# m96-chan/PyGPUkit

Measured on AMD Instinct MI355X. Metric: decode tokens/sec/GPU + prefill TFLOPS (% MFMA peak), Qwen3-0.6B bf16, higher is better.
Workload: dtype bf16

## Files before the change

include/pgk_hip.h:

```cpp
#ifndef PGK_HIP_H
#define PGK_HIP_H

#include <stddef.h>
#include <stdint.h>

#ifdef __cplusplus
extern "C" {
#endif

typedef int pgk_status;
#define PGK_OK 0
#define PGK_ERR_INVALID 1
#define PGK_ERR_HIP 2
#define PGK_ERR_UNSUPPORTED 3
#define PGK_ERR_RCCL 4
#define PGK_ERR_JIT 5

typedef enum {
    PGK_F64 = 0, PGK_F32 = 1, PGK_F16 = 2, PGK_BF16 = 3, PGK_I64 = 4,
    PGK_I32 = 5, PGK_I16 = 6, PGK_I8 = 7, PGK_U8 = 8, PGK_I4 = 9
} pgk_dtype;

typedef void* pgk_stream;
typedef void* pgk_event;
// ... 154 lines not shown
                             pgk_stream s);
pgk_status pgk_gemm_fp8_nt(const uint8_t* a_fp8, const float* a_scale, const uint8_t* w_fp8_nk, const void* w_scale,
                           void* c, int m, int n, int k, pgk_stream s);
pgk_status pgk_gemm_fp8_fp8_nn(const uint8_t* a_mk, const uint8_t* b_kn, uint8_t* d_mn, const float* scale_a,
                               const float* scale_b, int m, int n, int k, pgk_stream s);
pgk_status pgk_quantize_fp8_rows(const void* x, uint8_t* out_fp8, float* out_scale, int m, int k, pgk_dtype dt,
                                 pgk_stream s);
pgk_status pgk_quantize_fp8_blocks(const void* w_bf16, uint8_t* out_fp8, void* out_scale_bf16, int n, int k,
                                   pgk_stream s);

pgk_status pgk_quantize_nvf4(const void* x_kn, uint8_t* data, uint8_t* scale, int k, int n, pgk_stream s);
pgk_status pgk_quantize_nvf4_nk(const void* x_nk, uint8_t* data, uint8_t* scale, int n, int k, pgk_stream s);
size_t pgk_gemv_nvf4_workspace_bytes(int k, int n);
pgk_status pgk_gemv_nvf4_bf16(const void* a, const uint8_t* data, const uint8_t* scale, void* c, void* workspace, int k,
                              int n, float alpha, pgk_stream s);
pgk_status pgk_quantize_e2m1_unit(const void* x, uint8_t* out, int rows, int k, int transpose, pgk_stream s);
pgk_status pgk_gemm_fp4_nt(const uint8_t* a_packed, const uint8_t* b_packed, void* d, int m, int n, int kp, pgk_stream s);
size_t pgk_gemm_nvf4_workspace_bytes(int m, int n, int k);

pgk_status pgk_sdpa_causal(const void* q, const void* k, const void* v, void* out, int hq, int hkv, int q_len,
                           int kv_len, int d, float scale, int64_t q_stride_h, int64_t q_stride_s,
                           int64_t kv_stride_h, int64_t kv_stride_s, int64_t o_stride_h, int64_t o_stride_s,
                           pgk_dtype dt, pgk_stream s);
pgk_status pgk_sdpa_causal_fp8(const void* q, const void* k, const void* v, void* out, int hq, int hkv, int q_len,
                               int kv_len, int d, float scale, int64_t q_stride_h, int64_t q_stride_s,
                               int64_t kv_stride_h, int64_t kv_stride_s, int64_t o_stride_h, int64_t o_stride_s,
                               pgk_dtype dt, pgk_stream s);
pgk_status pgk_quantize_fp8_per_head(const void* x, uint8_t* codes, uint8_t* scale_bytes, int heads, int rows, int d,
                                     int64_t stride_h, int64_t stride_s, pgk_dtype dt, pgk_stream s);
pgk_status pgk_l2norm(const void* in, void* out, int rows, int features, float eps, pgk_dtype dt, pgk_stream s);
pgk_status pgk_irope_scale_q(const void* q, const void* positions, void* out, int seq_len, int n_heads, int head_dim,
                             float attn_scale, float floor_scale, pgk_dtype pos_dt, pgk_dtype dt, pgk_stream s);
pgk_status pgk_sdpa_irope(const void* q, const void* k, const void* v, const void* positions, void* out, int hq, int hkv,
                          int q_len, int kv_len, int d, float attn_scale, float floor_scale, int causal_offset,
                          int64_t q_stride_h, int64_t q_stride_s, int64_t kv_stride_h, int64_t kv_stride_s,
                          int64_t o_stride_h, int64_t o_stride_s, pgk_dtype pos_dt, pgk_dtype dt, pgk_stream s);
pgk_status pgk_llama4_qk_norm_cache_write(void* q, const void* k, const void* v, void* k_cache, void* v_cache, int seq, int hq,
                                          int hkv, int max_seq, int d, float eps, int qk_norm, int h_pos,
                                          const int32_t* pos_buf, pgk_dtype dt, pgk_stream s);
pgk_status pgk_sdpa_irope_fixed_cache(const void* q, const void* k_cache, const void* v_cache, void* out, int hq, int hkv,
                                      int max_seq, int d, float attn_scale, float floor_scale, int h_pos,
                                      const int32_t* pos_buf, void* workspace, pgk_dtype dt, pgk_stream s);
pgk_status pgk_pope_inplace(void* q, void* k, const void* encoding, int seq, int hq, int hk, int d, int start_pos, int max_seq,
                            pgk_dtype dt, pgk_stream s);
pgk_status pgk_alibi_compute_bias(const void* slopes, void* bias, int seq_len, int num_heads, int causal, pgk_stream s);
pgk_status pgk_alibi_add_bias(void* scores, const void* slopes, int batch, int num_heads, int q_len, int kv_len, int start_pos,
// ... 88 lines not shown
```

pygpukit_amd/_hip.py:

```python

from __future__ import annotations

import ctypes as C
import os

_HERE = os.path.dirname(os.path.abspath(__file__))
LIB_PATH = os.environ.get("PGK_LIB") or os.path.join(_HERE, "libpgk_hip.so")

c_void_pp = C.POINTER(C.c_void_p)
c_i32_p = C.POINTER(C.c_int32)


class PgkError(RuntimeError):
    """A libpgk_hip call returned a non-zero status (reference: std::runtime_error / CudaError
    surfacing as RuntimeError, native/core/types.hpp:108-111)."""


class DeviceProps(C.Structure):
    _fields_ = [("name", C.c_char * 128), ("arch", C.c_char * 32), ("total_mem", C.c_size_t),
                ("cu_count", C.c_int), ("wavefront_size", C.c_int), ("clock_khz", C.c_int),
                ("lds_per_cu", C.c_int), ("l2_bytes", C.c_int)]


class PoolStats(C.Structure):
# ... 47 lines not shown
    "pgk_argmax": [_V, _I, _I, _I, _V, _V],
    "pgk_gemm_nn": [_V, _V, _V, _I, _I, _I, _I, _V], "pgk_gemm_nt": [_V, _V, _V, _V, _I, _I, _I, _I, _V],
    "pgk_gemv": [_V, _V, _V, _I, _I, _I, _V], "pgk_gemv_fp8_bf16": [_V, _V, _V, _V, _I, _I, _I, _V],
    "pgk_w8a16_gemm_kn": [_V, _V, _V, _V, _I, _I, _I, _V], "pgk_w8a16_gemm_nk": [_V, _V, _V, _V, _I, _I, _I, _V],
    "pgk_gemm_fp8_nt": [_V, _V, _V, _V, _V, _I, _I, _I, _V], "pgk_gemm_fp8_fp8_nn": [_V, _V, _V, _V, _V, _I, _I, _I, _V],
    "pgk_quantize_fp8_rows": [_V, _V, _V, _I, _I, _I, _V],
    "pgk_quantize_fp8_blocks": [_V, _V, _V, _I, _I, _V],
    "pgk_quantize_nvf4": [_V, _V, _V, _I, _I, _V], "pgk_quantize_nvf4_nk": [_V, _V, _V, _I, _I, _V], "pgk_gemv_nvf4_bf16": [_V, _V, _V, _V, _V, _I, _I, _F, _V],
    "pgk_quantize_e2m1_unit": [_V, _V, _I, _I, _I, _V], "pgk_gemm_fp4_nt": [_V, _V, _V, _I, _I, _I, _V],
    "pgk_paged_attention_v1": [_V, _V, _V, _V, _V, _V, _I, _I, _I, _I, _I, _I, _I, _F, _V, _I, _V],
    "pgk_paged_cache_write": [_V, _V, _V, _V, _V, _I, _I, _I, _I, _I, _V],
    "pgk_scatter_last_token_logits": [_V, _V, _V, _V, _I, _I, _I, _V], "pgk_prepare_position_ids": [_V, _V, _V, _V, _V, _I, _V],
    "pgk_check_eos": [_V, _V, _I, _I, _V], "pgk_exclusive_cumsum_i32": [_V, _V, _I, _V],
    "pgk_st_open": [C.c_char_p, c_void_pp],
    "pgk_st_tensor_info": [_V, C.c_char_p, C.POINTER(_I), C.POINTER(_I), C.POINTER(_I64), C.POINTER(C.c_uint64), C.POINTER(C.c_uint64)],
    "pgk_st_tensor_data": [_V, C.c_char_p, c_void_pp, C.POINTER(C.c_uint64)], "pgk_st_upload": [_V, C.c_char_p, _V, C.c_uint64, _V],
    "pgk_jit_version": [C.POINTER(_I), C.POINTER(_I)],
    "pgk_jit_compile": [C.c_char_p, C.c_char_p, C.POINTER(C.c_char_p), _I, c_void_pp, C.POINTER(_I)],
    "pgk_jit_program_code": [_V, c_void_pp, C.POINTER(_Z)], "pgk_jit_kernel_create": [_V, C.c_char_p, c_void_pp, C.POINTER(_I)],
    "pgk_jit_suggested_block_size": [_V, _Z, C.POINTER(_I)],
    "pgk_jit_launch": [_V, C.c_uint, C.c_uint, C.c_uint, C.c_uint, C.c_uint, C.c_uint, C.c_uint, c_void_pp, _V],
    "pgk_sample_token": [_V, _I, _I, _I, _F, _I, _F, _F, _V, _V, _V],
    "pgk_sdpa_causal": [_V, _V, _V, _V, _I, _I, _I, _I, _I, _F, _I64, _I64, _I64, _I64, _I64, _I64, _I, _V],
    "pgk_sdpa_causal_fp8": [_V, _V, _V, _V, _I, _I, _I, _I, _I, _F, _I64, _I64, _I64, _I64, _I64, _I64, _I, _V],
    "pgk_quantize_fp8_per_head": [_V, _V, _V, _I, _I, _I, _I64, _I64, _I, _V], "pgk_device_arch": [C.POINTER(_I)],
    "pgk_l2norm": [_V, _V, _I, _I, _F, _I, _V], "pgk_irope_scale_q": [_V, _V, _V, _I, _I, _I, _F, _F, _I, _I, _V],
    "pgk_sdpa_irope": [_V, _V, _V, _V, _V, _I, _I, _I, _I, _I, _F, _F, _I, _I64, _I64, _I64, _I64, _I64, _I64, _I, _I, _V],
    "pgk_llama4_qk_norm_cache_write": [_V, _V, _V, _V, _V, _I, _I, _I, _I, _I, _F, _I, _I, _V, _I, _V],
    "pgk_sdpa_irope_fixed_cache": [_V, _V, _V, _V, _I, _I, _I, _I, _F, _F, _I, _V, _V, _I, _V],
    "pgk_sdpa_fixed_cache": [_V, _V, _V, _V, _I, _I, _I, _I, _I, _F, _I, _V, _V, _I, _V],
    "pgk_pope_inplace": [_V, _V, _V, _I, _I, _I, _I, _I, _I, _I, _V], "pgk_alibi_compute_bias": [_V, _V, _I, _I, _I, _V],
    "pgk_alibi_add_bias": [_V, _V, _I, _I, _I, _I, _I, _I, _I, _I, _V],
    "pgk_sdpa_alibi": [_V, _V, _V, _V, _V, _I, _I, _I, _I, _I, _F, _I64, _I64, _I64, _I64, _I64, _I64, _I, _V],
    "pgk_sdpa_alibi_fixed_cache": [_V, _V, _V, _V, _V, _I, _I, _I, _I, _I, _F, _I, _V, _V, _I, _V],
    "pgk_engine_create": [C.POINTER(ModelConfig), _V, _V, _V, C.POINTER(LayerWeights), c_void_pp],
    "pgk_engine_destroy": [_V], "pgk_engine_bytes": [_V, C.POINTER(_Z), C.POINTER(_Z)],
    "pgk_engine_prefill": [_V, _I, c_i32_p, _I, _I, _V, C.POINTER(_F), _V],
    "pgk_engine_set_state": [_V, c_i32_p, c_i32_p, _I, _V], "pgk_engine_decode_step": [_V, _I, _V],
    "pgk_engine_profile_step": [_V, _I, _I, C.POINTER(_F), C.POINTER(_I), _V],
    "pgk_engine_timeline": [_V, _I, _I, C.POINTER(C.c_uint64), _I, C.POINTER(_I), _V],
    "pgk_engine_capture": [_V, _I, _V], "pgk_engine_replay": [_V, _I, _V], "pgk_engine_logits_ptr": [_V, c_void_pp],
    "pgk_engine_read_tokens": [_V, c_i32_p, _I, _I, _V], "pgk_engine_reset_log": [_V, _V],
    "pgk_engine_set_sampling": [_V, _F, _I, _F, C.POINTER(_F), _I, _V],
    "pgk_engine_read_clock": [_V, C.POINTER(C.c_uint64), _I, _V],
    "pgk_engine_kv_ptr": [_V, _I, c_void_pp, c_void_pp], "pgk_engine_state_ptr": [_V, c_void_pp, c_void_pp], "pgk_engine_launches_per_step": [_V, C.POINTER(_I)],
    "pgk_moe_topk_softmax": [_V, _V, _V, _I, _I, _I, _I, _I, _V], "pgk_moe_softmax_topk": [_V, _I, _I, _I, _V],
# ... 75 lines not shown
```

pygpukit_amd/csrc/flash_common.hip.h:

```cpp
#pragma once

#include <type_traits>

#include "pgk_device.hip.h"
#include "pgk_internal.h"

namespace pgk {

typedef __bf16 bf16x8_fl __attribute__((ext_vector_type(8)));
typedef _Float16 f16x8_fl __attribute__((ext_vector_type(8)));
typedef float f32x16_fl __attribute__((ext_vector_type(16)));

template <class T> __device__ __forceinline__ f32x16_fl mfma32(const uint4& a, const uint4& b, f32x16_fl c);
template <> __device__ __forceinline__ f32x16_fl mfma32<bf16>(const uint4& a, const uint4& b, f32x16_fl c) {
    return __builtin_amdgcn_mfma_f32_32x32x16_bf16(__builtin_bit_cast(bf16x8_fl, a), __builtin_bit_cast(bf16x8_fl, b), c, 0, 0, 0);
}
template <> __device__ __forceinline__ f32x16_fl mfma32<f16>(const uint4& a, const uint4& b, f32x16_fl c) {
    return __builtin_amdgcn_mfma_f32_32x32x16_f16(__builtin_bit_cast(f16x8_fl, a), __builtin_bit_cast(f16x8_fl, b), c, 0, 0, 0);
}
template <class T> __device__ __forceinline__ uint32_t pack16x2(float lo, float hi);
template <> __device__ __forceinline__ uint32_t pack16x2<bf16>(float lo, float hi) { return pack_bf16x2(lo, hi); }
template <> __device__ __forceinline__ uint32_t pack16x2<f16>(float lo, float hi) {
    return (uint32_t)__builtin_bit_cast(uint16_t, static_cast<_Float16>(lo)) | ((uint32_t)__builtin_bit_cast(uint16_t, static_cast<_Float16>(hi)) << 16);
}
// ... 14 lines not shown
}

struct FlashPlain {};
struct FlashIrope {
    const void* positions;
    float attn_scale, floor_scale;
    int causal_offset;
    int pos_is_i64;
};
struct FlashAlibi {
    const float* slopes;
};

__device__ __forceinline__ int fl_v_off(int d, int c8) { return d * 128 + ((c8 ^ ((d >> 1) & 15)) << 3); }

struct FlashSplit {
    int nsplit;
    float* ml;
    void* o;
    uint8_t* q8;
    float* q8s;
};

inline int flash_nsplit(int nqt, int hq, int kv_len) {
    int nsplit = 1, dev = 0, cus = 256;
    hipDeviceProp_t prop;
    if (hipGetDevice(&dev) == hipSuccess && hipGetDeviceProperties(&prop, dev) == hipSuccess && prop.multiProcessorCount > 0) cus = prop.multiProcessorCount;
    const long long wgs = (long long)nqt * hq;
    while (nsplit < 4 && wgs * nsplit < 2LL * cus && ceil_div(kv_len, FL_BKV) >= 4 * (nsplit * 2)) nsplit *= 2;
    return nsplit;
}

template <class T, int D>
__global__ __launch_bounds__(256) void flash_merge_kernel(const float* ml, const T* po, T* out, int hq, int q_len, int nsplit, long long oh, long long os,
                                                          uint8_t* q8 = nullptr, float* q8s = nullptr) {
    constexpr int CPR = D / 8;
    const size_t gid = (size_t)blockIdx.x * 256 + threadIdx.x;
    const size_t nrow = (size_t)q_len * hq;
    if (gid >= nrow * CPR) return;
    const size_t rowi = gid / CPR;
    const int c = (int)(gid % CPR), qrow = (int)(rowi / hq), head = (int)(rowi % hq);
    float mstar = -INFINITY;
    for (int s2 = 0; s2 < nsplit; ++s2) mstar = fmaxf(mstar, ml[(((size_t)s2 * hq + head) * q_len + qrow) * 2]);
    float acc[8] = {0.f, 0.f, 0.f, 0.f, 0.f, 0.f, 0.f, 0.f}, den = 0.f;
    for (int s2 = 0; s2 < nsplit; ++s2) {
        const float* r = ml + (((size_t)s2 * hq + head) * q_len + qrow) * 2;
        const float w = (r[1] > 0.f) ? r[1] * __builtin_amdgcn_exp2f(r[0] - mstar) : 0.f;
        if (w > 0.f) {
            Vec<T> v;
            v.load(po + (((size_t)s2 * q_len + qrow) * hq + head) * D + c * 8);
            float f[8];
            v.to_float(f);
#pragma unroll
// ... 58 lines not shown
```

pygpukit_amd/csrc/ops_flash.hip:

```cpp

#include "flash_common.hip.h"

namespace pgk {

template <int D> __device__ __forceinline__ int fl_k_off(int r, int c) { return r * (2 * D) + ((c ^ (r & (D / 8 - 1))) << 4); }

template <class T, int D, class X = FlashPlain>
__global__ __launch_bounds__(FL_THREADS, 2) void flash_fwd_kernel(const T* q, const T* k, const T* vt, T* out, int hq, int hkv,
                                                              int q_len, int kv_len, int kv_pad, float scale_log2e, FlashStrides sd,
                                                              FlashSplit sp, X ex) {
    constexpr bool IROPE = std::is_same<X, FlashIrope>::value;
    constexpr bool ALIBI = std::is_same<X, FlashAlibi>::value;
    constexpr int NC = D / 8;
    constexpr int KS = D / 16;
    constexpr int DT = D / 32;
    constexpr int KCH = 64 * NC / FL_THREADS;
    constexpr int VCH = D * 8 / FL_THREADS;
    constexpr int K_BYTES = 64 * D * 2, V_BYTES = D * 128;
    extern __shared__ __attribute__((aligned(16))) char fl_smem[];
    auto Ks = [&](int buf) -> char* { return fl_smem + buf * K_BYTES; };
    auto Vs = [&](int buf) -> char* { return fl_smem + 2 * K_BYTES + buf * V_BYTES; };

    const int tid = threadIdx.x, lane = tid & 63, wid = tid >> 6, ql = lane & 31, h = lane >> 5;
    const int rep = hq / hkv, nqt = (q_len + FL_BQ - 1) / FL_BQ;
    const int id = blockIdx.x;
    const int kvh = id % hkv, rest = id / hkv;
    const int head = kvh * rep + rest % rep;
    const int rest2 = rest / rep;
    int order = rest2;
    const int nord = nqt * sp.nsplit;
    if (sp.nsplit > 1 && order >= nord / 2) order = nord / 2 + (nord - 1 - order);
    const int split = order % sp.nsplit;
    const int qt = nqt - 1 - order / sp.nsplit;
    const int qw0 = qt * FL_BQ + wid * 32;
    int mask_off = kv_len - q_len;
    if constexpr (IROPE) mask_off = ex.causal_offset;
    const int causal_off = mask_off;
    const T* qh = q + (size_t)head * sd.qh;
    const T* kh = k + (size_t)kvh * sd.kh;
    const T* vh = vt + (size_t)kvh * D * kv_pad;

    uint4 qf[KS];
    {
        const T* qrow = qh + (size_t)min(qw0 + ql, q_len - 1) * sd.qs + 8 * h;
        float qmul = scale_log2e;
        if constexpr (IROPE)
            qmul *= irope_temperature(irope_position(ex.positions, min(qw0 + ql, q_len - 1), ex.pos_is_i64), ex.attn_scale, ex.floor_scale);
#pragma unroll
        for (int ks = 0; ks < KS; ++ks) {
            Vec<T> v;
            v.load(qrow + ks * 16);
            float f[8];
            v.to_float(f);
#pragma unroll
            for (int j = 0; j < 8; ++j) f[j] *= qmul;
            v.from_float(f);
            qf[ks] = v.raw;
        }
    }
    f32x16_fl o[DT];
#pragma unroll
    for (int i = 0; i < DT; ++i)
#pragma unroll
        for (int r = 0; r < 16; ++r) o[i][r] = 0.f;
    float m_run = -INFINITY, l_run = 0.f;
    float slope2 = 0.f;
    if constexpr (ALIBI) slope2 = ex.slopes[head] * 1.4426950408889634f;

    const int q_last = min(qt * FL_BQ + FL_BQ - 1, q_len - 1);
    const int kv_end = min(kv_len, causal_off + q_last + 1);
    const int nt_all = (kv_end + FL_BKV - 1) / FL_BKV;
    const int t0 = (int)((long long)nt_all * split / sp.nsplit), t1 = (int)((long long)nt_all * (split + 1) / sp.nsplit);

    static_assert(KCH == VCH && (KCH == 2 || KCH == 4), "staging is written for D = 64 / 128");
    uint4 rk0, rk1, rk2, rk3, rv0, rv1, rv2, rv3;
    const int kr = tid / NC, kc16 = tid % NC;
    constexpr int KR_STEP = FL_THREADS / NC;
    const int vd = tid >> 3, vc = tid & 7;
    auto k_src = [&](int kv0, int i) { return kh + (size_t)min(kv0 + kr + KR_STEP * i, kv_len - 1) * sd.ks + kc16 * 8; };
    const uint32_t ko0 = (uint32_t)(kr * sd.ks + kc16 * 8), ko_step = (uint32_t)(KR_STEP * sd.ks);
    const uint32_t vo0 = (uint32_t)(vd * kv_pad + vc * 8), vo_step = (uint32_t)(32 * kv_pad);
    auto load_k = [&](int t) {
        const int kv0 = t * FL_BKV;
        if (kv0 + FL_BKV <= kv_len) {
            const T* kt = kh + (size_t)kv0 * sd.ks;
            rk0 = *reinterpret_cast<const uint4*>(kt + ko0);
            rk1 = *reinterpret_cast<const uint4*>(kt + ko0 + ko_step);
            if constexpr (KCH == 4) {
                rk2 = *reinterpret_cast<const uint4*>(kt + ko0 + 2 * ko_step);
                rk3 = *reinterpret_cast<const uint4*>(kt + ko0 + 3 * ko_step);
            }
        } else {
            rk0 = *reinterpret_cast<const uint4*>(k_src(kv0, 0));
            rk1 = *reinterpret_cast<const uint4*>(k_src(kv0, 1));
            if constexpr (KCH == 4) {
                rk2 = *reinterpret_cast<const uint4*>(k_src(kv0, 2));
                rk3 = *reinterpret_cast<const uint4*>(k_src(kv0, 3));
            }
        }
    };
    auto load_v = [&](int t) {
        const T* vtile = vh + t * FL_BKV;
        rv0 = *reinterpret_cast<const uint4*>(vtile + vo0);
        rv1 = *reinterpret_cast<const uint4*>(vtile + vo0 + vo_step);
        if constexpr (VCH == 4) {
            rv2 = *reinterpret_cast<const uint4*>(vtile + vo0 + 2 * vo_step);
            rv3 = *reinterpret_cast<const uint4*>(vtile + vo0 + 3 * vo_step);
        }
    };
    auto put_v = [&](char* base, int d, const uint4& x) {
        *reinterpret_cast<uint2*>(base + fl_v_off(d, 2 * vc)) = make_uint2(x.x, x.y);
        *reinterpret_cast<uint2*>(base + fl_v_off(d, 2 * vc + 1)) = make_uint2(x.z, x.w);
    };
    auto store_k = [&](int buf) {
        char* kb = Ks(buf);
        *reinterpret_cast<uint4*>(kb + fl_k_off<D>(kr, kc16)) = rk0;
        *reinterpret_cast<uint4*>(kb + fl_k_off<D>(kr + KR_STEP, kc16)) = rk1;
        if constexpr (KCH == 4) {
            *reinterpret_cast<uint4*>(kb + fl_k_off<D>(kr + 2 * KR_STEP, kc16)) = rk2;
            *reinterpret_cast<uint4*>(kb + fl_k_off<D>(kr + 3 * KR_STEP, kc16)) = rk3;
        }
    };
    auto store_v = [&](int buf) {
        char* vb = Vs(buf);
        put_v(vb, vd, rv0);
        put_v(vb, vd + 32, rv1);
        if constexpr (VCH == 4) {
            put_v(vb, vd + 64, rv2);
            put_v(vb, vd + 96, rv3);
        }
    };
    auto qk = [&](int buf, int kv0, f32x16_fl& s0, f32x16_fl& s1) {
        if constexpr (ALIBI) {
            const float base = slope2 * (float)(kv0 + 4 * h - (causal_off + qw0 + ql));
#pragma unroll
            for (int r = 0; r < 16; ++r) {
                s0[r] = fmaf(slope2, (float)((r & 3) + 8 * (r >> 2)), base);
                s1[r] = fmaf(slope2, (float)(32 + (r & 3) + 8 * (r >> 2)), base);
            }
        } else {
#pragma unroll
            for (int r = 0; r < 16; ++r) { s0[r] = 0.f; s1[r] = 0.f; }
        }
#pragma unroll
        for (int ks = 0; ks < KS; ++ks) {
            const uint4 a0 = *reinterpret_cast<const uint4*>(Ks(buf) + fl_k_off<D>(ql, 2 * ks + h));
            const uint4 a1 = *reinterpret_cast<const uint4*>(Ks(buf) + fl_k_off<D>(32 + ql, 2 * ks + h));
            s0 = mfma32<T>(a0, qf[ks], s0);
            s1 = mfma32<T>(a1, qf[ks], s1);
        }
    };
    auto live = [&](int t) -> bool { return t < t1 && t * FL_BKV <= causal_off + qw0 + 31; };

    f32x16_fl sc0, sc1;
    if (t0 < t1) {
        load_k(t0);
        load_v(t0);
        store_k(t0 & 1);
        store_v(t0 & 1);
    }
#pragma unroll
    for (int ks = 0; ks < KS; ++ks) asm volatile("" ::"v"(qf[ks].x), "v"(qf[ks].y), "v"(qf[ks].z), "v"(qf[ks].w));
    __syncthreads();
    typedef uint32_t fl_u32x2 __attribute__((ext_vector_type(2)));
    typedef __attribute__((address_space(3))) const volatile fl_u32x2* fl_lds_cv64;
    for (int t = t0; t < t1; ++t) {
        const int buf = t & 1, kv0 = t * FL_BKV;
        if (t + 1 < t1) { load_k(t + 1); load_v(t + 1); }
        const bool cur = live(t);
        if (cur) qk(buf, kv0, sc0, sc1);
        if (cur) {
            const bool need_mask = kv0 + FL_BKV - 1 > causal_off + qw0 || kv0 + FL_BKV > kv_len;
            const int lim = min(causal_off + qw0 + ql, kv_len - 1) - kv0 - 4 * h;
            float mx = -INFINITY;
            if (need_mask) {
#pragma unroll
                for (int r = 0; r < 16; ++r) {
                    const int kvl = (r & 3) + 8 * (r >> 2);
                    sc0[r] = kvl <= lim ? sc0[r] : -INFINITY;
                    sc1[r] = 32 + kvl <= lim ? sc1[r] : -INFINITY;
                }
            }
#pragma unroll
            for (int r = 0; r < 16; r += 2) mx = fmaxf(fmaxf(fmaxf(sc0[r], sc1[r]), fmaxf(sc0[r + 1], sc1[r + 1])), mx);
            mx = fmaxf(mx, __shfl_xor(mx, 32, 64));
            const float m_new = (mx > m_run + 6.0f || m_run == -INFINITY) ? fmaxf(m_run, mx) : m_run;
            const float m_use = m_new == -INFINITY ? 0.f : m_new;
            const bool moved = __builtin_amdgcn_ballot_w64(m_new != m_run) != 0;
            const float alpha = moved ? __builtin_amdgcn_exp2f(m_run - m_use) : 1.0f;
            float ls = 0.f;
#pragma unroll
            for (int r = 0; r < 16; ++r) {
                sc0[r] = __builtin_amdgcn_exp2f(sc0[r] - m_use);
                sc1[r] = __builtin_amdgcn_exp2f(sc1[r] - m_use);
                ls += sc0[r] + sc1[r];
            }
            l_run = l_run * alpha + ls;
            m_run = m_new;
            if (moved) {
#pragma unroll
                for (int i = 0; i < DT; ++i)
#pragma unroll
                    for (int r = 0; r < 16; ++r) o[i][r] *= alpha;
            }
            const char* vrow = Vs(buf) + ql * 128;
            const int vsw = (ql >> 1) & 15;
#pragma unroll
            for (int s = 0; s < 4; ++s) {
                uint4 pb;
                if (s < 2) {
                    pb = make_uint4(pack16x2<T>(sc0[8 * s + 0], sc0[8 * s + 1]), pack16x2<T>(sc0[8 * s + 2], sc0[8 * s + 3]),
                                    pack16x2<T>(sc0[8 * s + 4], sc0[8 * s + 5]), pack16x2<T>(sc0[8 * s + 6], sc0[8 * s + 7]));
                } else {
                    pb = make_uint4(pack16x2<T>(sc1[8 * (s - 2) + 0], sc1[8 * (s - 2) + 1]), pack16x2<T>(sc1[8 * (s - 2) + 2], sc1[8 * (s - 2) + 3]),
                                    pack16x2<T>(sc1[8 * (s - 2) + 4], sc1[8 * (s - 2) + 5]), pack16x2<T>(sc1[8 * (s - 2) + 6], sc1[8 * (s - 2) + 7]));
                }
#pragma unroll
                for (int i = 0; i < DT; ++i) {
                    const fl_u32x2 lo = *(fl_lds_cv64)(vrow + (((4 * s + h) ^ vsw) << 3) + i * 4096);
                    const fl_u32x2 hi = *(fl_lds_cv64)(vrow + (((4 * s + 2 + h) ^ vsw) << 3) + i * 4096);
                    o[i] = mfma32<T>(make_uint4(lo.x, lo.y, hi.x, hi.y), pb, o[i]);
                }
            }
        }
        if (t + 1 < t1) { store_k(buf ^ 1); store_v(buf ^ 1); }
        __syncthreads();
    }

    const float l_tot = l_run + __shfl_xor(l_run, 32, 64);
    const float inv = l_tot > 0.f ? 1.f / l_tot : 0.f;
    const int qrow = qw0 + ql;
    if constexpr (std::is_same<T, bf16>::value && D == 128 && std::is_same<X, FlashPlain>::value) {
        if (sp.q8 != nullptr && sp.nsplit == 1) {
            float amax = 0.f;
#pragma unroll
            for (int i = 0; i < DT; ++i)
#pragma unroll
                for (int e = 0; e < 16; ++e) {
                    o[i][e] = __uint_as_float(pack_bf16x2(o[i][e] * inv, 0.f) << 16);
                    amax = fmaxf(amax, fabsf(o[i][e]));
                }
            amax = fmaxf(amax, __shfl_xor(amax, 32, 64));
            const float sc = amax > 0.f ? amax / 448.0f : 1.0f;
            if (qrow < q_len) {
                uint8_t* qrow8 = sp.q8 + ((size_t)qrow * hq + head) * D;
#pragma unroll
                for (int i = 0; i < DT; ++i)
#pragma unroll
                    for (int g = 0; g < 4; ++g)
                        *reinterpret_cast<uint32_t*>(qrow8 + i * 32 + 8 * g + 4 * h) =
                            pack_fp8x4(o[i][4 * g] / sc, o[i][4 * g + 1] / sc, o[i][4 * g + 2] / sc, o[i][4 * g + 3] / sc);
                if (h == 0) sp.q8s[(size_t)qrow * hq + head] = sc;
            }
            return;
        }
    }
    if (qrow < q_len) {
        T* orow = sp.nsplit > 1 ? reinterpret_cast<T*>(sp.o) + (((size_t)split * q_len + qrow) * hq + head) * D
                                : out + (size_t)head * sd.oh + (size_t)qrow * sd.os;
#pragma unroll
        for (int i = 0; i < DT; ++i)
#pragma unroll
            for (int g = 0; g < 4; ++g) {
                uint2 w;
                w.x = pack16x2<T>(o[i][4 * g] * inv, o[i][4 * g + 1] * inv);
                w.y = pack16x2<T>(o[i][4 * g + 2] * inv, o[i][4 * g + 3] * inv);
                *reinterpret_cast<uint2*>(orow + i * 32 + 8 * g + 4 * h) = w;
            }
        if (sp.nsplit > 1 && h == 0) {
            float* ml = sp.ml + (((size_t)split * hq + head) * q_len + qrow) * 2;
            ml[0] = m_run;
            ml[1] = l_tot;
        }
    }
}

template <class T, int D, class X = FlashPlain>
static pgk_status flash_launch(const T* q, const T* k, const T* v, T* out, int hq, int hkv, int q_len, int kv_len, float scale,
                               const FlashStrides& sd, hipStream_t st, uint8_t* q8 = nullptr, float* q8s = nullptr, X ex = X{},
                               int kv_seen = 0) {
    const int kv_pad = ceil_div(kv_len, 64) * 64;
    const int nqt = ceil_div(q_len, FL_BQ);
    const int nsplit = flash_nsplit(nqt, hq, kv_seen > 0 ? kv_seen : kv_len);
    const size_t vt_bytes = (size_t)hkv * D * kv_pad * sizeof(T);
    const size_t po_bytes = nsplit > 1 ? (size_t)nsplit * q_len * hq * D * sizeof(T) : 0;
    const size_t ml_bytes = nsplit > 1 ? (size_t)nsplit * hq * q_len * 2 * sizeof(float) : 0;
    void* ws = nullptr;
    if (pgk_status r = pgk_malloc(&ws, vt_bytes + po_bytes + ml_bytes + 512)) return r;
    char* base = (char*)ws;
    T* vt = (T*)base;
    FlashSplit sp{nsplit, nullptr, nullptr, q8, q8s};
    if (nsplit > 1) {
        sp.o = base + ((vt_bytes + 255) & ~(size_t)255);
        sp.ml = (float*)((char*)sp.o + ((po_bytes + 255) & ~(size_t)255));
    }
    transpose_v_kernel<T, D><<<dim3(kv_pad / 64, hkv), 256, 0, st>>>(v, vt, kv_len, kv_pad, sd.kh, sd.ks);
    constexpr size_t LDS = 2 * (size_t)(64 * D * 2) + 2 * (size_t)(D * 128);
    static bool attr_done = false;
    if (LDS > 48 * 1024 && !attr_done) {
        PGK_CHECK_HIP(hipFuncSetAttribute(reinterpret_cast<const void*>(&flash_fwd_kernel<T, D, X>),
                                          hipFuncAttributeMaxDynamicSharedMemorySize, (int)LDS));
        attr_done = true;
    }
    flash_fwd_kernel<T, D, X><<<nqt * hq * nsplit, FL_THREADS, LDS, st>>>(q, k, (const T*)vt, out, hq, hkv, q_len, kv_len, kv_pad,
                                                                         scale * 1.4426950408889634f, sd, sp, ex);
    hipError_t e = hipGetLastError();
    if (e == hipSuccess && nsplit > 1) {
        const size_t work = (size_t)q_len * hq * (D / 8);
        flash_merge_kernel<T, D><<<(unsigned)((work + 255) / 256), 256, 0, st>>>(sp.ml, (const T*)sp.o, out, hq, q_len, nsplit, sd.oh, sd.os, q8, q8s);
        e = hipGetLastError();
    }
    pgk_free(ws);
    PGK_CHECK_HIP(e);
    return PGK_OK;
}

pgk_status flash_prefill(const void* q, const void* k, const void* v, void* out, int hq, int hkv, int q_len, int kv_len, int d,
                         float scale, long long qh, long long qs, long long kh, long long ks, long long oh, long long os,
                         int dt16, hipStream_t st) {
    const FlashStrides sd{qh, qs, kh, ks, oh, os};
    if (dt16 == 0) {
        if (d == 128) return flash_launch<bf16, 128>((const bf16*)q, (const bf16*)k, (const bf16*)v, (bf16*)out, hq, hkv, q_len, kv_len, scale, sd, st);
        return flash_launch<bf16, 64>((const bf16*)q, (const bf16*)k, (const bf16*)v, (bf16*)out, hq, hkv, q_len, kv_len, scale, sd, st);
    }
    if (d == 128) return flash_launch<f16, 128>((const f16*)q, (const f16*)k, (const f16*)v, (f16*)out, hq, hkv, q_len, kv_len, scale, sd, st);
    return flash_launch<f16, 64>((const f16*)q, (const f16*)k, (const f16*)v, (f16*)out, hq, hkv, q_len, kv_len, scale, sd, st);
}

pgk_status flash_prefill_irope(const void* q, const void* k, const void* v, const void* positions, void* out, int hq, int hkv, int q_len,
                               int kv_len, int d, float attn_scale, float floor_scale, int causal_offset, long long qh, long long qs,
                               long long kh, long long ks, long long oh, long long os, int pos_is_i64, int dt16, hipStream_t st) {
    const FlashStrides sd{qh, qs, kh, ks, oh, os};
    const int off = causal_offset < kv_len ? causal_offset : kv_len;
    const FlashIrope ex{positions, attn_scale, floor_scale, off, pos_is_i64};
    const float scale = 1.0f / sqrtf((float)d);
    const int kv_seen = (long long)off + q_len < kv_len ? off + q_len : kv_len;
#define PGK_IROPE_CASE(T, DD) \
    return flash_launch<T, DD, FlashIrope>((const T*)q, (const T*)k, (const T*)v, (T*)out, hq, hkv, q_len, kv_len, scale, sd, st, nullptr, nullptr, ex, kv_seen)
    if (dt16 == 0) {
        if (d == 128) PGK_IROPE_CASE(bf16, 128);
        PGK_IROPE_CASE(bf16, 64);
    }
    if (d == 128) PGK_IROPE_CASE(f16, 128);
    PGK_IROPE_CASE(f16, 64);
#undef PGK_IROPE_CASE
}

pgk_status flash_prefill_alibi(const void* q, const void* k, const void* v, const float* slopes, void* out, int hq, int hkv, int q_len,
                               int kv_len, int d, float scale, long long qh, long long qs, long long kh, long long ks, long long oh,
                               long long os, int dt16, hipStream_t st) {
    const FlashStrides sd{qh, qs, kh, ks, oh, os};
    const FlashAlibi ex{slopes};
#define PGK_ALIBI_CASE(T, DD) \
    return flash_launch<T, DD, FlashAlibi>((const T*)q, (const T*)k, (const T*)v, (T*)out, hq, hkv, q_len, kv_len, scale, sd, st, nullptr, nullptr, ex)
    if (dt16 == 0) {
        if (d == 128) PGK_ALIBI_CASE(bf16, 128);
        PGK_ALIBI_CASE(bf16, 64);
    }
    if (d == 128) PGK_ALIBI_CASE(f16, 128);
    PGK_ALIBI_CASE(f16, 64);
#undef PGK_ALIBI_CASE
}

pgk_status flash_prefill_q8(const void* q, const void* k, const void* v, uint8_t* q8, float* q8s, int hq, int hkv, int q_len, int kv_len,
                            float scale, long long qh, long long qs, long long kh, long long ks, hipStream_t st) {
    PGK_REQUIRE(q8 && q8s && q_len > 128, "flash_prefill_q8: needs output buffers and q_len > 128 (got %d)", q_len);
    const FlashStrides sd{qh, qs, kh, ks, 0, 0};
    return flash_launch<bf16, 128>((const bf16*)q, (const bf16*)k, (const bf16*)v, nullptr, hq, hkv, q_len, kv_len, scale, sd, st, q8, q8s);
}

}
```

Baseline: 1676.

## Balance flash prefill work with per-tile KV runs and drop the V transpose

After: 1677, median of 2. Within noise of the previous version (+0.1%).

```diff
diff --git a/include/pgk_hip.h b/include/pgk_hip.h
--- a/include/pgk_hip.h
+++ b/include/pgk_hip.h
@@ -200,6 +200,7 @@
                            int kv_len, int d, float scale, int64_t q_stride_h, int64_t q_stride_s,
                            int64_t kv_stride_h, int64_t kv_stride_s, int64_t o_stride_h, int64_t o_stride_s,
                            pgk_dtype dt, pgk_stream s);
+pgk_status pgk_flash_run_plan(int hq, int q_len, int kv_len, int* run_tiles, int* cut_tiles, int* runs_per_head);
 pgk_status pgk_sdpa_causal_fp8(const void* q, const void* k, const void* v, void* out, int hq, int hkv, int q_len,
                                int kv_len, int d, float scale, int64_t q_stride_h, int64_t q_stride_s,
                                int64_t kv_stride_h, int64_t kv_stride_s, int64_t o_stride_h, int64_t o_stride_s,
diff --git a/pygpukit_amd/_hip.py b/pygpukit_amd/_hip.py
--- a/pygpukit_amd/_hip.py
+++ b/pygpukit_amd/_hip.py
@@ -93,6 +93,7 @@
     "pgk_jit_launch": [_V, C.c_uint, C.c_uint, C.c_uint, C.c_uint, C.c_uint, C.c_uint, C.c_uint, c_void_pp, _V],
     "pgk_sample_token": [_V, _I, _I, _I, _F, _I, _F, _F, _V, _V, _V],
     "pgk_sdpa_causal": [_V, _V, _V, _V, _I, _I, _I, _I, _I, _F, _I64, _I64, _I64, _I64, _I64, _I64, _I, _V],
+    "pgk_flash_run_plan": [_I, _I, _I, C.POINTER(_I), C.POINTER(_I), C.POINTER(_I)],
     "pgk_sdpa_causal_fp8": [_V, _V, _V, _V, _I, _I, _I, _I, _I, _F, _I64, _I64, _I64, _I64, _I64, _I64, _I, _V],
     "pgk_quantize_fp8_per_head": [_V, _V, _V, _I, _I, _I, _I64, _I64, _I, _V], "pgk_device_arch": [C.POINTER(_I)],
     "pgk_l2norm": [_V, _V, _I, _I, _F, _I, _V], "pgk_irope_scale_q": [_V, _V, _V, _I, _I, _I, _F, _F, _I, _I, _V],
diff --git a/pygpukit_amd/csrc/flash_common.hip.h b/pygpukit_amd/csrc/flash_common.hip.h
--- a/pygpukit_amd/csrc/flash_common.hip.h
+++ b/pygpukit_amd/csrc/flash_common.hip.h
@@ -60,13 +60,140 @@
     float* q8s;
 };
 
+inline int flash_cu_count() {
+    static int cached[64] = {};
+    int dev = 0, n = 0;
+    if (hipGetDevice(&dev) != hipSuccess || dev < 0 || dev >= 64) dev = 0;
+    if (cached[dev] > 0) return cached[dev];
+    if (hipDeviceGetAttribute(&n, hipDeviceAttributeMultiprocessorCount, dev) != hipSuccess || n <= 0) return 256;
+    cached[dev] = n;
+    return n;
+}
+
 inline int flash_nsplit(int nqt, int hq, int kv_len) {
-    int nsplit = 1, dev = 0, cus = 256;
-    hipDeviceProp_t prop;
-    if (hipGetDevice(&dev) == hipSuccess && hipGetDeviceProperties(&prop, dev) == hipSuccess && prop.multiProcessorCount > 0) cus = prop.multiProcessorCount;
+    int nsplit = 1;
+    const int cus = flash_cu_count();
     const long long wgs = (long long)nqt * hq;
     while (nsplit < 4 && wgs * nsplit < 2LL * cus && ceil_div(kv_len, FL_BKV) >= 4 * (nsplit * 2)) nsplit *= 2;
     return nsplit;
+}
+
+template <int D> __device__ __forceinline__ int fl_vr_off(int r, int ch) {
+    if constexpr (D == 128) return r * 256 + ((ch ^ (((r & 3) << 2) | ((r >> 2) & 3))) << 4);
+    else return r * 128 + ((ch ^ ((((r >> 1) & 1) << 2) | ((r >> 2) & 3))) << 4);
+}
+
+struct FlashRuns {
+    int R;
+    uint32_t rinv;
+    int nst, nrs, nr;
+    float* ml;
+    void* o;
+    uint8_t* q8;
+    float* q8s;
+    int ntab;
+    uint32_t tab[64];
+};
+constexpr int FL_TAB = 64;
+__host__ __device__ __forceinline__ int fl_nt_all(int qt, int q_len, int kv_len, int mask_off) {
+    const int q_last = qt * FL_BQ + FL_BQ - 1 < q_len - 1 ? qt * FL_BQ + FL_BQ - 1 : q_len - 1;
+    const int kv_end = kv_len < mask_off + q_last + 1 ? kv_len : mask_off + q_last + 1;
+    return (kv_end + FL_BKV - 1) / FL_BKV;
+}
+__host__ __device__ __forceinline__ int fl_nruns(int nt, int R, uint32_t rinv) {
+    return (int)(((unsigned long long)(uint32_t)(nt + R - 1) * rinv) >> 32);
+}
+constexpr int FL_RUN_MIN = 6;
+constexpr int FL_RUN_MAX = 1 << 13;
+
+inline FlashRuns flash_runs(int hq, int q_len, int kv_len, int mask_off, int force_r = 0) {
+    const int nqt = ceil_div(q_len, FL_BQ);
+    long long tiles = 0;
+    for (int qt = 0; qt < nqt; ++qt) tiles += fl_nt_all(qt, q_len, kv_len, mask_off);
+    const int cus = flash_cu_count();
+    long long r = (tiles * hq * 7 + 10LL * cus - 1) / (10LL * cus);
+    if (force_r > 0) r = force_r;
+    FlashRuns fr{};
+    fr.R = (int)(r < FL_RUN_MIN ? FL_RUN_MIN : r > FL_RUN_MAX ? FL_RUN_MAX : r);
+    fr.rinv = (uint32_t)(((1ull << 32) + fr.R - 1) / fr.R);
+    for (int qt = nqt - 1; qt >= 0; --qt) {
+        const int n = fl_nruns(fl_nt_all(qt, q_len, kv_len, mask_off), fr.R, fr.rinv);
+        fr.nr += n;
+        if (n > 1) { fr.nst += 1; fr.nrs += n; }
+    }
+    if (fr.nst > 0 && fr.nr <= FL_TAB) {
+        int len[FL_TAB], slot = 0;
+        for (int qt = nqt - 1; qt >= 0; --qt) {
+            const int nt = fl_nt_all(qt, q_len, kv_len, mask_off), n = fl_nruns(nt, fr.R, fr.rinv);
+            for (int i = 0; i < n; ++i, ++slot) {
+                const int l = (int)((long long)nt * (i + 1) / n) - (int)((long long)nt * i / n);
+                int at = fr.ntab++;
+                for (; at > 0 && len[at - 1] < l; --at) { len[at] = len[at - 1]; fr.tab[at] = fr.tab[at - 1]; }
+                len[at] = l;
+                fr.tab[at] = (uint32_t)qt | (uint32_t)i << 10 | (uint32_t)n << 16 | (uint32_t)(n > 1 ? slot : 0) << 22;
+            }
+        }
+        const long long wgs = (long long)hq * fr.nr;
+        if (wgs > cus && wgs <= 2LL * cus && cus % hq == 0)
+            for (int a = cus / hq, b = fr.nr - 1; a < b; ++a, --b) { const uint32_t t = fr.tab[a]; fr.tab[a] = fr.tab[b]; fr.tab[b] = t; }
+    }
+    return fr;
+}
+
+template <class T, int D>
+__global__ __launch_bounds__(256) void flash_merge_runs_kernel(T* out, int hq, int q_len, int kv_len, int mask_off, FlashRuns fr, long long oh, long long os) {
+    constexpr int CPR = D / 8, BPT = FL_BQ * CPR / 256;
+    const int nqt = (q_len + FL_BQ - 1) / FL_BQ;
+    const int ti = blockIdx.x / BPT, head = blockIdx.y;
+    int first = 0;
+    for (int j = 0; j < ti; ++j) first += fl_nruns(fl_nt_all(nqt - 1 - j, q_len, kv_len, mask_off), fr.R, fr.rinv);
+    const int qt = nqt - 1 - ti;
+    const int nrun = fl_nruns(fl_nt_all(qt, q_len, kv_len, mask_off), fr.R, fr.rinv);
+    const int idx = (blockIdx.x % BPT) * 256 + threadIdx.x;
+    const int r = idx / CPR, c = idx % CPR, qrow = qt * FL_BQ + r;
+    if (qrow >= q_len) return;
+    const size_t rec0 = (size_t)head * fr.nrs + first;
+    const float* ml = fr.ml + (rec0 * FL_BQ + r) * 2;
+    const T* po = reinterpret_cast<const T*>(fr.o) + (rec0 * FL_BQ + r) * D + c * 8;
+    float mstar = -INFINITY;
+    for (int s2 = 0; s2 < nrun; ++s2) mstar = fmaxf(mstar, ml[(size_t)s2 * FL_BQ * 2]);
+    float acc[8] = {0.f, 0.f, 0.f, 0.f, 0.f, 0.f, 0.f, 0.f}, den = 0.f;
+    for (int s2 = 0; s2 < nrun; ++s2) {
+        const float* rr = ml + (size_t)s2 * FL_BQ * 2;
+        const float w = (rr[1] > 0.f) ? rr[1] * __builtin_amdgcn_exp2f(rr[0] - mstar) : 0.f;
+        if (w > 0.f) {
+            Vec<T> v;
+            v.load(po + (size_t)s2 * FL_BQ * D);
+            float f[8];
+            v.to_float(f);
+#pragma unroll
+            for (int j = 0; j < 8; ++j) acc[j] = fmaf(w, f[j], acc[j]);
+            den += w;
+        }
+    }
+    const float inv = den > 0.f ? 1.f / den : 0.f;
+#pragma unroll
+    for (int j = 0; j < 8; ++j) acc[j] *= inv;
+    Vec<T> v;
+    v.from_float(acc);
+    if constexpr (std::is_same<T, bf16>::value && D == 128) {
+        if (fr.q8 != nullptr) {
+            v.to_float(acc);
+            float amax = 0.f;
+#pragma unroll
+            for (int j = 0; j < 8; ++j) amax = fmaxf(amax, fabsf(acc[j]));
+            amax = group16_max(amax);
+            const float sc = amax > 0.f ? amax / 448.0f : 1.0f;
+            uint2 o8;
+            o8.x = pack_fp8x4(acc[0] / sc, acc[1] / sc, acc[2] / sc, acc[3] / sc);
+            o8.y = pack_fp8x4(acc[4] / sc, acc[5] / sc, acc[6] / sc, acc[7] / sc);
+            const size_t rowi = (size_t)qrow * hq + head;
+            *reinterpret_cast<uint2*>(fr.q8 + rowi * D + c * 8) = o8;
+            if (c == 0) fr.q8s[rowi] = sc;
+            return;
+        }
+    }
+    v.store(out + (size_t)head * oh + (size_t)qrow * os + c * 8);
 }
 
 template <class T, int D>
diff --git a/pygpukit_amd/csrc/ops_flash.hip b/pygpukit_amd/csrc/ops_flash.hip
--- a/pygpukit_amd/csrc/ops_flash.hip
+++ b/pygpukit_amd/csrc/ops_flash.hip
@@ -6,17 +6,16 @@
 template <int D> __device__ __forceinline__ int fl_k_off(int r, int c) { return r * (2 * D) + ((c ^ (r & (D / 8 - 1))) << 4); }
 
 template <class T, int D, class X = FlashPlain>
-__global__ __launch_bounds__(FL_THREADS, 2) void flash_fwd_kernel(const T* q, const T* k, const T* vt, T* out, int hq, int hkv,
-                                                              int q_len, int kv_len, int kv_pad, float scale_log2e, FlashStrides sd,
-                                                              FlashSplit sp, X ex) {
+__global__ __launch_bounds__(FL_THREADS, 2) void flash_fwd_kernel(const T* q, const T* k, const T* v, T* out, int hq, int hkv,
+                                                              int q_len, int kv_len, float scale_log2e, FlashStrides sd,
+                                                              FlashRuns sp, X ex) {
     constexpr bool IROPE = std::is_same<X, FlashIrope>::value;
     constexpr bool ALIBI = std::is_same<X, FlashAlibi>::value;
     constexpr int NC = D / 8;
     constexpr int KS = D / 16;
     constexpr int DT = D / 32;
     constexpr int KCH = 64 * NC / FL_THREADS;
-    constexpr int VCH = D * 8 / FL_THREADS;
-    constexpr int K_BYTES = 64 * D * 2, V_BYTES = D * 128;
+    constexpr int K_BYTES = 64 * D * 2, V_BYTES = 64 * D * 2;
     extern __shared__ __attribute__((aligned(16))) char fl_smem[];
     auto Ks = [&](int buf) -> char* { return fl_smem + buf * K_BYTES; };
     auto Vs = [&](int buf) -> char* { return fl_smem + 2 * K_BYTES + buf * V_BYTES; };
@@ -26,19 +25,26 @@
     const int id = blockIdx.x;
     const int kvh = id % hkv, rest = id / hkv;
     const int head = kvh * rep + rest % rep;
-    const int rest2 = rest / rep;
-    int order = rest2;
-    const int nord = nqt * sp.nsplit;
-    if (sp.nsplit > 1 && order >= nord / 2) order = nord / 2 + (nord - 1 - order);
-    const int split = order % sp.nsplit;
-    const int qt = nqt - 1 - order / sp.nsplit;
-    const int qw0 = qt * FL_BQ + wid * 32;
+    const int order = rest / rep;
     int mask_off = kv_len - q_len;
     if constexpr (IROPE) mask_off = ex.causal_offset;
     const int causal_off = mask_off;
+    int qt = nqt - 1 - sp.nst - (order - sp.nrs), split = 0, nsplit = 1, slot = order;
+    if (sp.ntab > 0) {
+        const uint32_t e = sp.tab[order];
+        qt = (int)(e & 1023u);
+        split = (int)(e >> 10 & 63u);
+        nsplit = (int)(e >> 16 & 63u);
+        slot = (int)(e >> 22);
+    } else if (order < sp.nrs) {
+        qt = nqt - 1;
+        split = order;
+        while ((nsplit = fl_nruns(fl_nt_all(qt, q_len, kv_len, causal_off), sp.R, sp.rinv)) <= split) { split -= nsplit; --qt; }
+    }
+    const int qw0 = qt * FL_BQ + wid * 32;
     const T* qh = q + (size_t)head * sd.qh;
     const T* kh = k + (size_t)kvh * sd.kh;
-    const T* vh = vt + (size_t)kvh * D * kv_pad;
+    const T* vh = v + (size_t)kvh * sd.kh;
 
     uint4 qf[KS];
     {
@@ -67,19 +73,16 @@
     float slope2 = 0.f;
     if constexpr (ALIBI) slope2 = ex.slopes[head] * 1.4426950408889634f;
 
-    const int q_last = min(qt * FL_BQ + FL_BQ - 1, q_len - 1);
-    const int kv_end = min(kv_len, causal_off + q_last + 1);
-    const int nt_all = (kv_end + FL_BKV - 1) / FL_BKV;
-    const int t0 = (int)((long long)nt_all * split / sp.nsplit), t1 = (int)((long long)nt_all * (split + 1) / sp.nsplit);
-
-    static_assert(KCH == VCH && (KCH == 2 || KCH == 4), "staging is written for D = 64 / 128");
+    const int nt_all = fl_nt_all(qt, q_len, kv_len, causal_off);
+    const int t0 = (int)((long long)nt_all * split / nsplit), t1 = (int)((long long)nt_all * (split + 1) / nsplit);
+
+    static_assert(KCH == 2 || KCH == 4, "staging is written for D = 64 / 128");
     uint4 rk0, rk1, rk2, rk3, rv0, rv1, rv2, rv3;
     const int kr = tid / NC, kc16 = tid % NC;
     constexpr int KR_STEP = FL_THREADS / NC;
-    const int vd = tid >> 3, vc = tid & 7;
     auto k_src = [&](int kv0, int i) { return kh + (size_t)min(kv0 + kr + KR_STEP * i, kv_len - 1) * sd.ks + kc16 * 8; };
+    auto v_src = [&](int kv0, int i) { return vh + (size_t)min(kv0 + kr + KR_STEP * i, kv_len - 1) * sd.ks + kc16 * 8; };
     const uint32_t ko0 = (uint32_t)(kr * sd.ks + kc16 * 8), ko_step = (uint32_t)(KR_STEP * sd.ks);
-    const uint32_t vo0 = (uint32_t)(vd * kv_pad + vc * 8), vo_step = (uint32_t)(32 * kv_pad);
     auto load_k = [&](int t) {
         const int kv0 = t * FL_BKV;
         if (kv0 + FL_BKV <= kv_len) {
@@ -100,17 +103,23 @@
         }
     };
     auto load_v = [&](int t) {
-        const T* vtile = vh + t * FL_BKV;
-        rv0 = *reinterpret_cast<const uint4*>(vtile + vo0);
-        rv1 = *reinterpret_cast<const uint4*>(vtile + vo0 + vo_step);
-        if constexpr (VCH == 4) {
-            rv2 = *reinterpret_cast<const uint4*>(vtile + vo0 + 2 * vo_step);
-            rv3 = *reinterpret_cast<const uint4*>(vtile + vo0 + 3 * vo_step);
-        }
-    };
-    auto put_v = [&](char* base, int d, const uint4& x) {
-        *reinterpret_cast<uint2*>(base + fl_v_off(d, 2 * vc)) = make_uint2(x.x, x.y);
-        *reinterpret_cast<uint2*>(base + fl_v_off(d, 2 * vc + 1)) = make_uint2(x.z, x.w);
+        const int kv0 = t * FL_BKV;
+        if (kv0 + FL_BKV <= kv_len) {
+            const T* vtile = vh + (size_t)kv0 * sd.ks;
+            rv0 = *reinterpret_cast<const uint4*>(vtile + ko0);
+            rv1 = *reinterpret_cast<const uint4*>(vtile + ko0 + ko_step);
+            if constexpr (KCH == 4) {
+                rv2 = *reinterpret_cast<const uint4*>(vtile + ko0 + 2 * ko_step);
+                rv3 = *reinterpret_cast<const uint4*>(vtile + ko0 + 3 * ko_step);
+            }
+        } else {
+            rv0 = *reinterpret_cast<const uint4*>(v_src(kv0, 0));
+            rv1 = *reinterpret_cast<const uint4*>(v_src(kv0, 1));
+            if constexpr (KCH == 4) {
+                rv2 = *reinterpret_cast<const uint4*>(v_src(kv0, 2));
+                rv3 = *reinterpret_cast<const uint4*>(v_src(kv0, 3));
+            }
+        }
     };
     auto store_k = [&](int buf) {
         char* kb = Ks(buf);
@@ -123,11 +132,11 @@
     };
     auto store_v = [&](int buf) {
         char* vb = Vs(buf);
-        put_v(vb, vd, rv0);
-        put_v(vb, vd + 32, rv1);
-        if constexpr (VCH == 4) {
-            put_v(vb, vd + 64, rv2);
-            put_v(vb, vd + 96, rv3);
+        *reinterpret_cast<uint4*>(vb + fl_vr_off<D>(kr, kc16)) = rv0;
+        *reinterpret_cast<uint4*>(vb + fl_vr_off<D>(kr + KR_STEP, kc16)) = rv1;
+        if constexpr (KCH == 4) {
+            *reinterpret_cast<uint4*>(vb + fl_vr_off<D>(kr + 2 * KR_STEP, kc16)) = rv2;
+            *reinterpret_cast<uint4*>(vb + fl_vr_off<D>(kr + 3 * KR_STEP, kc16)) = rv3;
         }
     };
     auto qk = [&](int buf, int kv0, f32x16_fl& s0, f32x16_fl& s1) {
@@ -162,8 +171,16 @@
 #pragma unroll
     for (int ks = 0; ks < KS; ++ks) asm volatile("" ::"v"(qf[ks].x), "v"(qf[ks].y), "v"(qf[ks].z), "v"(qf[ks].w));
     __syncthreads();
-    typedef uint32_t fl_u32x2 __attribute__((ext_vector_type(2)));
-    typedef __attribute__((address_space(3))) const volatile fl_u32x2* fl_lds_cv64;
+    typedef short fl_v4s __attribute__((ext_vector_type(4)));
+    typedef __attribute__((address_space(3))) fl_v4s* fl_lds_v4s;
+    uint32_t vl[2][DT];
+    {
+        const int li = lane & 15, tq = li >> 2, tp = li & 3, gl = (lane >> 4) & 1;
+#pragma unroll
+        for (int u = 0; u < 2; ++u)
+#pragma unroll
+            for (int i = 0; i < DT; ++i) vl[u][i] = (uint32_t)(fl_vr_off<D>(8 * u + 4 * h + tq, 4 * i + 2 * gl + (tp >> 1)) + 8 * (tp & 1));
+    }
     for (int t = t0; t < t1; ++t) {
         const int buf = t & 1, kv0 = t * FL_BKV;
         if (t + 1 < t1) { load_k(t + 1); load_v(t + 1); }
@@ -203,8 +220,7 @@
 #pragma unroll
                     for (int r = 0; r < 16; ++r) o[i][r] *= alpha;
             }
-            const char* vrow = Vs(buf) + ql * 128;
-            const int vsw = (ql >> 1) & 15;
+            const char* vb = Vs(buf);
 #pragma unroll
             for (int s = 0; s < 4; ++s) {
                 uint4 pb;
@@ -217,8 +233,8 @@
                 }
 #pragma unroll
                 for (int i = 0; i < DT; ++i) {
-                    const fl_u32x2 lo = *(fl_lds_cv64)(vrow + (((4 * s + h) ^ vsw) << 3) + i * 4096);
-                    const fl_u32x2 hi = *(fl_lds_cv64)(vrow + (((4 * s + 2 + h) ^ vsw) << 3) + i * 4096);
+                    const uint2 lo = __builtin_bit_cast(uint2, __builtin_amdgcn_ds_read_tr16_b64_v4i16((fl_lds_v4s)(vb + vl[0][i] + s * (16 * 2 * D))));
+                    const uint2 hi = __builtin_bit_cast(uint2, __builtin_amdgcn_ds_read_tr16_b64_v4i16((fl_lds_v4s)(vb + vl[1][i] + s * (16 * 2 * D))));
                     o[i] = mfma32<T>(make_uint4(lo.x, lo.y, hi.x, hi.y), pb, o[i]);
                 }
             }
@@ -231,7 +247,7 @@
     const float inv = l_tot > 0.f ? 1.f / l_tot : 0.f;
     const int qrow = qw0 + ql;
     if constexpr (std::is_same<T, bf16>::value && D == 128 && std::is_same<X, FlashPlain>::value) {
-        if (sp.q8 != nullptr && sp.nsplit == 1) {
+        if (sp.q8 != nullptr && nsplit == 1) {
             float amax = 0.f;
 #pragma unroll
             for (int i = 0; i < DT; ++i)
@@ -256,8 +272,8 @@
         }
     }
     if (qrow < q_len) {
-        T* orow = sp.nsplit > 1 ? reinterpret_cast<T*>(sp.o) + (((size_t)split * q_len + qrow) * hq + head) * D
-                                : out + (size_t)head * sd.oh + (size_t)qrow * sd.os;
+        const size_t rec = ((size_t)head * sp.nrs + slot) * FL_BQ + (qrow - qt * FL_BQ);
+        T* orow = nsplit > 1 ? reinterpret_cast<T*>(sp.o) + rec * D : out + (size_t)head * sd.oh + (size_t)qrow * sd.os;
 #pragma unroll
         for (int i = 0; i < DT; ++i)
 #pragma unroll
@@ -267,50 +283,52 @@
                 w.y = pack16x2<T>(o[i][4 * g + 2] * inv, o[i][4 * g + 3] * inv);
                 *reinterpret_cast<uint2*>(orow + i * 32 + 8 * g + 4 * h) = w;
             }
-        if (sp.nsplit > 1 && h == 0) {
-            float* ml = sp.ml + (((size_t)split * hq + head) * q_len + qrow) * 2;
+        if (nsplit > 1 && h == 0) {
+            float* ml = sp.ml + rec * 2;
             ml[0] = m_run;
             ml[1] = l_tot;
         }
     }
 }
 
+static int flash_force_r() {
+    static const int v = [] { const char* e = getenv("PGK_FLASH_RUN_TILES"); return e ? atoi(e) : 0; }();
+    return v;
+}
+
 template <class T, int D, class X = FlashPlain>
 static pgk_status flash_launch(const T* q, const T* k, const T* v, T* out, int hq, int hkv, int q_len, int kv_len, float scale,
-                               const FlashStrides& sd, hipStream_t st, uint8_t* q8 = nullptr, float* q8s = nullptr, X ex = X{},
-                               int kv_seen = 0) {
-    const int kv_pad = ceil_div(kv_len, 64) * 64;
+                               const FlashStrides& sd, hipStream_t st, uint8_t* q8 = nullptr, float* q8s = nullptr, X ex = X{}) {
     const int nqt = ceil_div(q_len, FL_BQ);
-    const int nsplit = flash_nsplit(nqt, hq, kv_seen > 0 ? kv_seen : kv_len);
-    const size_t vt_bytes = (size_t)hkv * D * kv_pad * sizeof(T);
-    const size_t po_bytes = nsplit > 1 ? (size_t)nsplit * q_len * hq * D * sizeof(T) : 0;
-    const size_t ml_bytes = nsplit > 1 ? (size_t)nsplit * hq * q_len * 2 * sizeof(float) : 0;
+    int mask_off = kv_len - q_len;
+    if constexpr (std::is_same<X, FlashIrope>::value) mask_off = ex.causal_offset;
+    FlashRuns fr = flash_runs(hq, q_len, kv_len, mask_off, flash_force_r());
+    fr.q8 = q8;
+    fr.q8s = q8s;
     void* ws = nullptr;
-    if (pgk_status r = pgk_malloc(&ws, vt_bytes + po_bytes + ml_bytes + 512)) return r;
-    char* base = (char*)ws;
-    T* vt = (T*)base;
-    FlashSplit sp{nsplit, nullptr, nullptr, q8, q8s};
-    if (nsplit > 1) {
-        sp.o = base + ((vt_bytes + 255) & ~(size_t)255);
-        sp.ml = (float*)((char*)sp.o + ((po_bytes + 255) & ~(size_t)255));
-    }
-    transpose_v_kernel<T, D><<<dim3(kv_pad / 64, hkv), 256, 0, st>>>(v, vt, kv_len, kv_pad, sd.kh, sd.ks);
-    constexpr size_t LDS = 2 * (size_t)(64 * D * 2) + 2 * (size_t)(D * 128);
+    if (fr.nrs > 0) {
+        const size_t po_bytes = ((size_t)hq * fr.nrs * FL_BQ * D * sizeof(T) + 255) & ~(size_t)255;
+        const size_t ml_bytes = (size_t)hq * fr.nrs * FL_BQ * 2 * sizeof(float);
+        if (pgk_status r = pgk_malloc(&ws, po_bytes + ml_bytes)) return r;
+        fr.o = ws;
+        fr.ml = (float*)((char*)ws + po_bytes);
+    }
+    constexpr size_t LDS = 4 * (size_t)(64 * D * 2);
     static bool attr_done = false;
+    hipError_t e = hipSuccess;
     if (LDS > 48 * 1024 && !attr_done) {
-        PGK_CHECK_HIP(hipFuncSetAttribute(reinterpret_cast<const void*>(&flash_fwd_kernel<T, D, X>),
-                                          hipFuncAttributeMaxDynamicSharedMemorySize, (int)LDS));
-        attr_done = true;
-    }
-    flash_fwd_kernel<T, D, X><<<nqt * hq * nsplit, FL_THREADS, LDS, st>>>(q, k, (const T*)vt, out, hq, hkv, q_len, kv_len, kv_pad,
-                                                                         scale * 1.4426950408889634f, sd, sp, ex);
-    hipError_t e = hipGetLastError();
-    if (e == hipSuccess && nsplit > 1) {
-        const size_t work = (size_t)q_len * hq * (D / 8);
-        flash_merge_kernel<T, D><<<(unsigned)((work + 255) / 256), 256, 0, st>>>(sp.ml, (const T*)sp.o, out, hq, q_len, nsplit, sd.oh, sd.os, q8, q8s);
+        e = hipFuncSetAttribute(reinterpret_cast<const void*>(&flash_fwd_kernel<T, D, X>), hipFuncAttributeMaxDynamicSharedMemorySize, (int)LDS);
+        attr_done = e == hipSuccess;
+    }
+    if (e == hipSuccess) {
+        flash_fwd_kernel<T, D, X><<<hq * fr.nr, FL_THREADS, LDS, st>>>(q, k, v, out, hq, hkv, q_len, kv_len, scale * 1.4426950408889634f, sd, fr, ex);
         e = hipGetLastError();
     }
-    pgk_free(ws);
+    if (e == hipSuccess && fr.nst > 0) {
+        flash_merge_runs_kernel<T, D><<<dim3(fr.nst * (FL_BQ * (D / 8) / 256), hq), 256, 0, st>>>(out, hq, q_len, kv_len, mask_off, fr, sd.oh, sd.os);
+        e = hipGetLastError();
+    }
+    if (ws) pgk_free(ws);
     PGK_CHECK_HIP(e);
     return PGK_OK;
 }
@@ -334,9 +352,8 @@
     const int off = causal_offset < kv_len ? causal_offset : kv_len;
     const FlashIrope ex{positions, attn_scale, floor_scale, off, pos_is_i64};
     const float scale = 1.0f / sqrtf((float)d);
-    const int kv_seen = (long long)off + q_len < kv_len ? off + q_len : kv_len;
 #define PGK_IROPE_CASE(T, DD) \
-    return flash_launch<T, DD, FlashIrope>((const T*)q, (const T*)k, (const T*)v, (T*)out, hq, hkv, q_len, kv_len, scale, sd, st, nullptr, nullptr, ex, kv_seen)
+    return flash_launch<T, DD, FlashIrope>((const T*)q, (const T*)k, (const T*)v, (T*)out, hq, hkv, q_len, kv_len, scale, sd, st, nullptr, nullptr, ex)
     if (dt16 == 0) {
         if (d == 128) PGK_IROPE_CASE(bf16, 128);
         PGK_IROPE_CASE(bf16, 64);
@@ -370,3 +387,12 @@
 }
 
 }
+
+extern "C" pgk_status pgk_flash_run_plan(int hq, int q_len, int kv_len, int* run_tiles, int* cut_tiles, int* runs_per_head) {
+    PGK_REQUIRE(hq > 0 && q_len > 0 && kv_len >= q_len, "pgk_flash_run_plan: bad shape hq=%d q_len=%d kv_len=%d", hq, q_len, kv_len);
+    const pgk::FlashRuns fr = pgk::flash_runs(hq, q_len, kv_len, kv_len - q_len, pgk::flash_force_r());
+    if (run_tiles) *run_tiles = fr.R;
+    if (cut_tiles) *cut_tiles = fr.nst;
+    if (runs_per_head) *runs_per_head = fr.nr;
+    return PGK_OK;
+}
```
